# qwerfdsaplking/SATrans

Hardware: AMD Instinct MI355X
Metric: training samples/sec (AliCCP-shaped, emb=32, 3L/4H, meta_mode=QK) (higher is better)
Workload: dtype f32; 1 GPU; BASELINE configs[1]: AliCCP-shaped SATrans training step, 19 fields, 6,571,961 table rows (841 MB fp32), uniform ids, dropout on, dense-Adam+L2 semantics over all rows; batch_per_gpu=8192, global_batch=8192, embedding_dim=32, layers=3, heads=4, fields=19, parallelism=dp1

## Files before the change

include/satrans_hip.h:

```cpp
#ifndef SATRANS_HIP_H
#define SATRANS_HIP_H

#include <stdint.h>

#ifdef __cplusplus
extern "C" {
#endif

#define SATRANS_ABI_VERSION 7

#define SATRANS_OK 0
#define SATRANS_E_BADARG (-1)
#define SATRANS_E_UNSUPPORTED (-2)
#define SATRANS_E_LAUNCH (-3)
#define SATRANS_E_WORKSPACE (-4)

#define SATRANS_ID_F32 0
#define SATRANS_ID_I32 1
#define SATRANS_ID_I64 2

#define SATRANS_META_Q 1
#define SATRANS_META_K 2
#define SATRANS_RELU_OUT 4
#define SATRANS_NO_RES 8
// ... 129 lines not shown
    int64_t tab_stride;
    const float* x;
    const int32_t *order, *seg;
    const float *tab, *ln_g, *ln_b;
} satrans_metanet_desc;
int64_t satrans_metanet_saved_floats(const satrans_metanet_desc* d);
int64_t satrans_metanet_scratch_floats(const satrans_metanet_desc* d);
int satrans_metanet_fwd(const satrans_metanet_desc* d, float* y, float* saved, void* stream);
int satrans_metanet_bwd(const satrans_metanet_desc* d, const float* dy, float* dx, const float* saved, float* scratch,
                        float* g_tab, float* g_ln, void* stream);

int64_t satrans_layer_bwd_slab_floats(const satrans_layer_desc* d);
int satrans_layer_bwd(const satrans_layer_desc* d, const float* dy, float* dx, float* slabs,
                      float* g_wq, float* g_wk, float* g_wv, float* g_wo, float* g_ln, float* g_lnq,
                      float* g_lnk, float* g_tab_q, float* g_tab_k, void* stream);

int satrans_head(const float* a, const float* dense, int64_t dense_stride, const int32_t* dense_cols, int n_dense,
                 int B, int FD, const float* w, const float* bias, float* prob, float* logit, const float* y,
                 double* loss_sum, float* da, float* g_w, float* g_b, float* scratch, void* stream);

#define SATRANS_LOSS_BCE 0
#define SATRANS_LOSS_MSE 1
#define SATRANS_LOSS_MAE 2
int satrans_head_loss(const float* a, const float* dense, int64_t dense_stride, const int32_t* dense_cols, int n_dense, int B,
                      int FD, const float* w, const float* bias, float* prob, float* logit, const float* y, double* loss_sum,
                      float* da, float* g_w, float* g_b, float* scratch, int loss_kind, void* stream);

typedef struct satrans_head_desc {
    const float* w;
    const float* bias;
// ... 70 lines not shown
int satrans_embed_mark_touched(const int32_t* sorted_rows, int64_t n, int64_t total_rows, uint32_t* touched,
                               void* stream);

int satrans_embed_segment_sums(const int32_t* sorted_rows, const int32_t* src, int64_t n, const float* gemb, int D,
                               float* partial_ws, double* reg_partials, float* g_rows, void* stream);
int64_t satrans_embed_adam_rows_partials(int64_t rows, int D);
int satrans_embed_adam_rows(float* arena, float* m, float* v, int32_t* last, int64_t row0, int64_t rows, int D,
                            const float* g_rows, const satrans_adam_hparams* h, int t, double* reg_partials,
                            void* stream);
int satrans_embed_pack_rows(const int32_t* src, int64_t n, const float* gemb, int D, float* out, void* stream);

int64_t satrans_embed_lazy_reg_partials(int64_t n, int D);
int satrans_embed_lazy_replay(float* arena, float* m, float* v, int32_t* last, int D, const int32_t* sorted_rows,
                              int64_t n, int target, const double* table, const satrans_adam_hparams* h,
                              double* reg_partials, void* stream);
int satrans_embed_lazy_flush(float* arena, float* m, float* v, int32_t* last, int64_t total_rows, int D, int target,
                             const double* table, const satrans_adam_hparams* h, int64_t n, double* reg_partials,
                             void* stream);
int satrans_embed_lazy_mark(const int32_t* sorted_rows, int64_t n, int32_t* last, int t, void* stream);

int satrans_debug_check_packed_math(int mode, uint64_t first, uint64_t count, uint64_t* mismatches, void* stream);

int satrans_embed_grad_dense(const float* arena, const int32_t* sorted_rows, const int32_t* src, int64_t n,
                             const float* gemb, int64_t total_rows, int D, float l2, float* g_arena,
                             void* stream);

int satrans_sum_f64(const double* v, int64_t count, double* out, int accumulate, void* stream);

int64_t satrans_attn_stats_workspace_bytes(int B, int H, int F, int K);
int satrans_attn_stats_accumulate(const float* att, const int32_t* key, int B, int H, int F, int K, double* acc,
// ... 40 lines not shown
```

satrans_amd/csrc/capi.hip:

```cpp
#include <stdarg.h>
#include <stdlib.h>
#include <string.h>

#include "common.h"

namespace satrans {
static thread_local char g_error[512] = "";
void set_error(const char* fmt, ...) {
    va_list ap;
    va_start(ap, fmt);
    vsnprintf(g_error, sizeof(g_error), fmt, ap);
    va_end(ap);
}
static int g_layer_impl = -1;
}

extern "C" {

int satrans_layer_validate(const satrans_layer_desc* d, const char* who);
int satrans_layer_fused_supported(const satrans_layer_desc* d);
int satrans_layer_fwd_fused(const satrans_layer_desc* d, float* y, float* att, void* stream);
int satrans_layer_fwd_lds(const satrans_layer_desc* d, float* y, float* att, void* stream);
int satrans_layer_bwd_fused_supported(const satrans_layer_desc* d);
int64_t satrans_layer_bwd_slab_floats_fused(const satrans_layer_desc* d);
int64_t satrans_layer_attn_save_floats_fused(const satrans_layer_desc* d);
int satrans_layer_bwd_fused(const satrans_layer_desc* d, const float* dy, float* dx, float* slabs, float* g_wq, float* g_wk,
                            float* g_wv, float* g_wo, float* g_ln, float* g_lnq, float* g_lnk, float* g_tab_q,
                            float* g_tab_k, void* stream);
int64_t satrans_layer_bwd_slab_floats_lds(const satrans_layer_desc* d);
int satrans_layer_bwd_lds(const satrans_layer_desc* d, const float* dy, float* dx, float* slabs, float* g_wq, float* g_wk,
                          float* g_wv, float* g_wo, float* g_ln, float* g_lnq, float* g_lnk, float* g_tab_q,
                          float* g_tab_k, void* stream);

int satrans_layer_bwd_head_fused_supported(const satrans_layer_desc* d, const satrans_head_desc* h);
int64_t satrans_layer_bwd_head_scratch_floats_fused(const satrans_layer_desc* d, int n_dense);
int satrans_layer_bwd_head_fused(const satrans_layer_desc* d, const satrans_head_desc* h, float* dx, float* slabs, float* g_wq,
                                 float* g_wk, float* g_wv, float* g_wo, float* g_ln, float* g_lnq, float* g_lnk, float* g_tab_q,
                                 float* g_tab_k, void* stream);

// ... 48 lines not shown
                    "layer_fwd: SATRANS_X_SORTED / SATRANS_Y_SORTED are flags of the general path (satrans_layer_fwd_generic)");
    if (satrans_layer_impl() == 0 && satrans_layer_fused_supported(d)) return satrans_layer_fwd_fused(d, y, att, stream);
    return satrans_layer_fwd_lds(d, y, att, stream);
}

int64_t satrans_layer_bwd_slab_floats(const satrans_layer_desc* d) {
    if (satrans_layer_validate(d, "layer_bwd")) return -1;
    int64_t n = satrans_layer_bwd_slab_floats_lds(d);
    if (satrans_layer_bwd_fused_supported(d)) {
        const int64_t f = satrans_layer_bwd_slab_floats_fused(d);
        if (f > n) n = f;
    }
    return n;
}

int64_t satrans_layer_attn_save_floats(const satrans_layer_desc* d) {
    if (satrans_layer_validate(d, "layer_attn_save")) return -1;
    if (satrans_layer_impl() != 0 || !satrans_layer_fused_supported(d) || !satrans_layer_bwd_fused_supported(d)) return 0;
    return satrans_layer_attn_save_floats_fused(d);
}

int satrans_layer_bwd(const satrans_layer_desc* d, const float* dy, float* dx, float* slabs, float* g_wq, float* g_wk,
                      float* g_wv, float* g_wo, float* g_ln, float* g_lnq, float* g_lnk, float* g_tab_q, float* g_tab_k,
                      void* stream) {
    int rc = satrans_layer_validate(d, "layer_bwd");
    if (rc) return rc;
    SATRANS_REQUIRE(!(d->flags & (SATRANS_X_SORTED | SATRANS_Y_SORTED)), SATRANS_E_UNSUPPORTED,
                    "layer_bwd: SATRANS_X_SORTED / SATRANS_Y_SORTED are flags of the general path (satrans_layer_bwd_generic)");
    if (satrans_layer_impl() == 0 && satrans_layer_bwd_fused_supported(d))
        return satrans_layer_bwd_fused(d, dy, dx, slabs, g_wq, g_wk, g_wv, g_wo, g_ln, g_lnq, g_lnk, g_tab_q, g_tab_k, stream);
// ... 57 lines not shown
```

satrans_amd/csrc/embed_adam.hip:

```cpp
#include <algorithm>
#include <cstdlib>
#include <cstring>

#include <rocprim/rocprim.hpp>

#include "common.h"

namespace satrans {

constexpr int kChunk = 16;
constexpr int kStreamBlock = 256;
constexpr int kStreamBlocks = 2048;

struct AdamK {
    float neg_step, w1, beta2, w2, eps, l2x2, l2;
    double rbc2;
    float rbc2f;
    int fast;
};

__host__ inline AdamK make_adamk(const satrans_adam_hparams& h) {
    AdamK k;
    k.neg_step = -h.lr_over_bc1;
    k.rbc2 = 1.0 / (double)h.bc2_sqrt;
// ... 621 lines not shown
                reg = replay_element4(p, m, v, from, target, table, k);
                P[at] = p; M[at] = m; V[at] = v;
            }
        }
    }
    __syncthreads();
    if (j < n && c == 0) {
        const int32_t row = sorted_rows[j];
        if ((j == 0 || sorted_rows[j - 1] != row) && last[row] < target) last[row] = target;
    }
    const double total = block_sum(reg, s_red);
    if (threadIdx.x == 0) {
        reg_partials[blockIdx.x] = total;
        for (int64_t t = (int64_t)blockIdx.x + gridDim.x; t < slots; t += gridDim.x) reg_partials[t] = 0.0;
    }
}

template <int D>
__global__ __launch_bounds__(256) void lazy_flush_kernel(float4* __restrict__ P, float4* __restrict__ M, float4* __restrict__ V,
                                                        int32_t* __restrict__ last, int64_t total_rows, int target,
                                                        const double2* __restrict__ table, LazyK k,
                                                        double* __restrict__ reg_partials) {
    constexpr int LR = D / 4;
    __shared__ double s_red[256];
    double reg = 0.0;
    const int64_t groups_per_pass = (int64_t)gridDim.x * 256 / LR;
    const int c = threadIdx.x % LR;
    for (int64_t row = ((int64_t)blockIdx.x * 256 + threadIdx.x) / LR; row < total_rows; row += groups_per_pass) {
        const int from = last[row];
        if (from < target) {
// ... 630 lines not shown
    hipStream_t stream = (hipStream_t)stream_;
    SATRANS_REQUIRE(arena && m && v && last && sorted_rows && table && h && reg_partials, SATRANS_E_BADARG,
                    "embed_lazy_replay: null pointer");
    SATRANS_REQUIRE(n > 0 && target >= 0, SATRANS_E_BADARG, "embed_lazy_replay: n=%lld target=%d", (long long)n, target);
    const LazyK k = make_lazyk(*h);
    SATRANS_REQUIRE(D % 4 == 0, SATRANS_E_UNSUPPORTED, "embed_lazy_replay: embedding_dim %d is not a multiple of 4", D);
    const int64_t slots = ceil_div(n * D, 256);
    const int64_t blocks = ceil_div(n * (D / 4), 256);
    DISPATCH_D(D, (lazy_replay_kernel<DD><<<(unsigned)blocks, 256, 0, stream>>>((float4*)arena, (float4*)m, (float4*)v, last,
                                                                                sorted_rows, n, target, (const double2*)table, k,
                                                                                reg_partials, slots)));
    SATRANS_CHECK_LAUNCH("lazy_replay_kernel");
    return SATRANS_OK;
}

extern "C" int satrans_embed_lazy_flush(float* arena, float* m, float* v, int32_t* last, int64_t total_rows, int D,
                                        int target, const double* table, const satrans_adam_hparams* h, int64_t n,
                                        double* reg_partials, void* stream_) {
    hipStream_t stream = (hipStream_t)stream_;
    SATRANS_REQUIRE(arena && m && v && last && table && h && reg_partials, SATRANS_E_BADARG, "embed_lazy_flush: null pointer");
    const LazyK k = make_lazyk(*h);
    double* reg = reg_partials + ceil_div(n * D, 256);
    DISPATCH_D(D, (lazy_flush_kernel<DD><<<kFlushBlocks, 256, 0, stream>>>((float4*)arena, (float4*)m, (float4*)v, last, total_rows,
                                                                          target, (const double2*)table, k, reg)));
    SATRANS_CHECK_LAUNCH("lazy_flush_kernel");
    return SATRANS_OK;
}

extern "C" int satrans_debug_check_packed_math(int mode, uint64_t first, uint64_t count, uint64_t* mismatches, void* stream_) {
    hipStream_t stream = (hipStream_t)stream_;
// ... 53 lines not shown
```

satrans_amd/csrc/layer_fused.hip:

```cpp
#include <hip/hip_ext.h>

#include "layer_fused_common.h"

namespace satrans {

struct KernelTimer {
    static constexpr int kPairs = 512;
    struct Pair { hipEvent_t start, stop; int kind; };
    Pair pairs[kPairs];
    int made = 0, used = 0;
    bool armed = false;
    Pair* next(int kind) {
        if (!armed || used >= kPairs) return nullptr;
        if (used >= made) {
            if (hipEventCreate(&pairs[made].start) != hipSuccess || hipEventCreate(&pairs[made].stop) != hipSuccess) return nullptr;
            ++made;
        }
        pairs[used].kind = kind;
        return &pairs[used++];
    }
};
static KernelTimer g_ktimer;

#ifdef SATRANS_DIAG_FWDSAVE
// ... 1943 lines not shown
    const int LD = D + 4, LU = U + 4;
    auto r4 = [](int64_t v) { return (v + 3) & ~(int64_t)3; };
    const int64_t tasks = (int64_t)T * H * F;
    const int copies = tr ? 2 : 1;
    const int64_t dd = (int64_t)D * LD;
    const int64_t mlp = (int64_t)D * LU + (int64_t)U * LD;
    const int64_t hd = head ? r4((int64_t)F * D + kHeadDenseMax) + 64 + 64 + 128 + (int64_t)kFusedBlock * 4 * (D / 16) + 64 * kHeadDenseMax : 0;
    const int64_t FP = (F + 3) & ~3;
    const int64_t ds = std::max<int64_t>(std::max<int64_t>(tasks * F, 2 * (int64_t)T * F * D), (int64_t)T * H * FP * FP);
    return copies * 4 * dd + (same_tab ? 1 : 2) * copies * mlp + 6 * D + 5 * 64 * LD + 2 * r4(tasks) + r4(tasks * F) + r4(ds) + hd + 64;
}

static int fused_width(const satrans_layer_desc* d) { return d->D == 64 ? 16 : 2 * d->D; }

struct FusedBwdPlan {
    int T, G;
    size_t lds;
    bool tr;
};

static bool fused_bwd_plan(const satrans_layer_desc* d, FusedBwdPlan& p, bool head = false) {
    if (!satrans_layer_fused_supported(d) || d->D > 32 || d->F > 32) return false;
    const bool same_tab = d->tab_q == d->tab_k && d->lnq_g == d->lnk_g && d->lnq_b == d->lnk_b;
    p.T = 64 / d->F;
    p.tr = false;
    const int Uw = fused_width(d);
    p.lds = (size_t)fused_bwd_lds_floats(p.T, d->F, d->D, Uw, d->H, same_tab, p.tr, head) * 4;
    if (p.lds > 160 * 1024) return false;
    const int64_t tiles = ceil_div(d->B, p.T) + d->S;
    p.G = (int)std::max<int64_t>(1, std::min<int64_t>(tiles, cu_count()));
    return true;
}

template <int D, int U, int H, bool SAME, bool TR, int FT = 0, int MOD = 0, bool SAVE = false, bool HEADF = false>
static int launch_bwd(const satrans_layer_desc* d, const FusedBwdPlan& p, const float* dy, float* dx, float* slabs,
                      hipStream_t stream, const FusedHeadArgs* hd = nullptr) {
    static size_t attr_set = 0;
    if (p.lds > attr_set) {
        hipError_t e = hipFuncSetAttribute((const void*)layer_bwd_fused_kernel<D, U, H, SAME, TR, FT, MOD, SAVE, HEADF>,
                                           hipFuncAttributeMaxDynamicSharedMemorySize, (int)p.lds);
        SATRANS_REQUIRE(e == hipSuccess, SATRANS_E_LAUNCH, "layer_bwd(fused): LDS attribute: %s", hipGetErrorString(e));
        attr_set = p.lds;
    }
    if (KernelTimer::Pair* tp = g_ktimer.next(HEADF ? 2 : 1))
        hipExtLaunchKernelGGL((layer_bwd_fused_kernel<D, U, H, SAME, TR, FT, MOD, SAVE, HEADF>), dim3(p.G), dim3(kFusedBlock),
// ... 39 lines not shown

extern "C" int satrans_layer_bwd_fused_supported(const satrans_layer_desc* d) {
    FusedBwdPlan p;
    return d && fused_bwd_plan(d, p) ? 1 : 0;
}

extern "C" int64_t satrans_layer_attn_save_floats_fused(const satrans_layer_desc* d) {
    FusedBwdPlan p;
    if (!d || !fused_bwd_plan(d, p)) return 0;
    const bool alt = d->flags & (SATRANS_GATE | SATRANS_BILINEAR);
    if (d->D != 32 || (!alt && (d->U != 64 || !(d->flags & (SATRANS_META_Q | SATRANS_META_K))))) return 0;
    const int64_t HF = (int64_t)d->H * d->F;
    if (d->F > 32 || (d->F * HF) % 4 != 0) return 0;
    const int64_t FPs = (d->F + 3) & ~3;
    return (int64_t)d->B * ((int64_t)d->H * d->F * FPs + 2 * HF + (int64_t)d->F * d->D + (int64_t)d->F * (2 * d->D + 2));
}

extern "C" int64_t satrans_layer_bwd_slab_floats_fused(const satrans_layer_desc* d) {
    FusedBwdPlan p;
    if (!d) return -1;
    int64_t n = -1;
    if (fused_bwd_plan(d, p)) {
        const int64_t CSZ = 4 * (int64_t)d->D * d->D + 6 * d->D, TSZ = 4 * (int64_t)d->D * fused_width(d);
        n = std::max<int64_t>(n, (int64_t)p.G * CSZ + (int64_t)(p.G + d->S) * TSZ);
    }
    return n;
}

static int launch_fused_reduce(const satrans_layer_desc* d, const FusedBwdPlan& p, float* slabs, float* g_wq, float* g_wk,
                               float* g_wv, float* g_wo, float* g_ln, float* g_lnq, float* g_lnk, float* g_tab_q, float* g_tab_k,
// ... 229 lines not shown
```

satrans_amd/engine.py:

```python
from __future__ import annotations

import contextlib
import ctypes as C
import math
import os
from typing import Dict, List, Optional

import torch

from . import native as N
from .inputs import split_columns


from .engine_local import LocalStepMixin
from .engine_owner import OwnerStepMixin
from .engine_replicated import ReplicatedStepMixin
from .streams import _STREAMS, shared_stream as _shared_stream


class PathEngine(LocalStepMixin, ReplicatedStepMixin, OwnerStepMixin):
    def __init__(self, model):
        self.lib = N.lib()
        m = self.m = model
        self.dev = m.embedding_arena.device
# ... 142 lines not shown
        self._owner_world = 0
        self._replicas_stale = False
        self.reg_small = torch.zeros(1, dtype=torch.float64, device=self.dev)
        self.fuse_gather = not self.varlen
        self.fuse_head = True
        self.prefetch = True
        self.owner_prefetch = os.environ.get("SATRANS_OWNER_PREFETCH", "0") == "1"
        self.adam_arith = os.environ.get("SATRANS_ADAM_ARITH", "fast")
        if self.adam_arith not in ("fast", "exact"):
            raise ValueError(f"SATRANS_ADAM_ARITH={self.adam_arith!r}: 'fast' or 'exact'")
        self.untimed_phases = frozenset()
        self.prep_early = True
        self.defer_reduce = True
        self.side_tail = True
        self.preclear = True
        self._side_tail = None
        self._tail_done = None
        self._prep = None
        self.save_attention = True
        self.fwd_bf16 = os.environ.get("SATRANS_FWD_BF16", "0") == "1"
        self.force_split = os.environ.get("SATRANS_SPLIT_TABLES", "0") == "1"
        self.last_step = None
        self._hp_table = None
        self._hp_cfg = None
        self._lazy_pending = False

    def _stream(self):
        return N.stream_handle(self.dev)

    class _Phase:
# ... 677 lines not shown
                n = len(d_descs)
                descs_a = (C.POINTER(N.LayerDesc) * n)(*[C.pointer(d_) for d_ in d_descs])
                slabs_a = (C.c_void_p * n)(*d_slabs)
                grads_a = (N.LayerGrads * n)()
                for i_, gp in enumerate(d_grads):
                    for name_, v_ in zip(("g_wq", "g_wk", "g_wv", "g_wo", "g_ln", "g_lnq", "g_lnk", "g_tab_q", "g_tab_k"), gp):
                        setattr(grads_a[i_], name_, v_)
                with self.phase("layer_bwd_reduce"):
                    N.check(lib.satrans_layer_bwd_reduce(n, descs_a, slabs_a, grads_a, C.byref(d_head) if d_head is not None else None,
                                                         self._stream()), "satrans_layer_bwd_reduce")
            if modulated:
                with self.phase("scenario_bwd"):
                    self.scenario_tables_backward(g_tabs)

        fork = None
        if after_layers is not None or (side_tail and d_descs):
            fork = torch.cuda.Event()
            fork.record(torch.cuda.current_stream(self.dev))
        if after_layers is not None:
            after_layers(fork)
        self._last_fork = fork
        self._tail_done = None
        if side_tail and d_descs:
            main = torch.cuda.current_stream(self.dev)
            if self._side_tail is None:
                self._side_tail = _shared_stream(self.dev, "tail", lambda: torch.cuda.Stream(self.dev))
            self._side_tail.wait_event(fork)
            with torch.cuda.stream(self._side_tail):
                if clear_late and not precleared:
                    g_clear.zero_()
                finish()
                self._tail_done = torch.cuda.Event()
                self._tail_done.record(self._side_tail)
        else:
            if clear_late and not precleared:
# ... 14 lines not shown

    def _low_priority_stream(self, name: str = "low_priority"):
        def make():
            handle = C.c_void_p()
            with torch.cuda.device(self.dev):
                rc = self.lib.satrans_stream_create_low_priority(C.byref(handle))
            if rc == 0 and handle.value:
                return torch.cuda.ExternalStream(handle.value, device=self.dev)
            return None
        st = _shared_stream(self.dev, name, make)
        if st is not None or name != "low_priority":
            return st
        self.prep_early = False
        return _shared_stream(self.dev, "side", lambda: torch.cuda.Stream(self.dev))

    def _prepare_async(self, X_next, ws_cur_B, fork=None, defer_bucket=False):
        B = X_next.shape[0]
        ws = self.train_workspace(B, 1, False)
        if "prep_alt" not in ws:
            ws["prep_alt"] = {k: torch.empty_like(ws[k]) for k in self._PREP_KEYS}
        alt = ws["prep_alt"]
        main = torch.cuda.current_stream(self.dev)
        if self._side is None:
            self._side = self._low_priority_stream() if self.prep_early else \
                _shared_stream(self.dev, "side", lambda: torch.cuda.Stream(self.dev))
        if fork is None:
            fork = torch.cuda.Event()
            fork.record(main)
        self._side.wait_event(fork)
        with torch.cuda.stream(self._side):
            st = self._stream()
            f_, lo_, n_ = self._sort_fields
            N.check(self.lib.satrans_embed_rows_sort_fields(X_next.data_ptr(), N.id_dtype_of(X_next), X_next.stride(0),
                                                            self.cols.data_ptr(), self.row_span.data_ptr(), alt["rows"].data_ptr(),
                                                            B, self.F, f_, lo_, n_, alt["sorted_rows"].data_ptr(),
                                                            alt["src"].data_ptr(), self.status.data_ptr(), st),
                    "satrans_embed_rows_sort_fields(next)")
            sorted_ev = torch.cuda.Event()
            sorted_ev.record(self._side)
            done = None
            if not defer_bucket:
                self._bucket(X_next, alt)
                done = torch.cuda.Event()
                done.record(self._side)
        self._prep = dict(key=self._prep_key(X_next), X=X_next, B=B, done=done, sorted=sorted_ev)

    def _take_prepared(self, X, ws) -> bool:
        prep, self._prep = self._prep, None
        if prep is None:
            return False
        if prep["key"] != self._prep_key(X) or prep["B"] != X.shape[0] or "prep_alt" not in ws:
            torch.cuda.current_stream(self.dev).wait_event(prep["done"] or prep["sorted"])
            return False
        alt = ws["prep_alt"]
        for k in self._PREP_KEYS:
            ws[k], alt[k] = alt[k], ws[k]
        torch.cuda.current_stream(self.dev).wait_event(prep["sorted"])
        self._prep_rest = prep["done"] or prep["sorted"]
        return True

    def _join_prepared(self) -> None:
        ev, self._prep_rest = getattr(self, "_prep_rest", None), None
        if ev is not None:
            torch.cuda.current_stream(self.dev).wait_event(ev)

    def train_step(self, X: torch.Tensor, y: torch.Tensor, next_X: Optional[torch.Tensor] = None):
        from . import parallel
        X = self._prepare_input(X)
        y = y.reshape(-1).to(torch.float32).contiguous()
        B = X.shape[0]
        self._ensure_train_state()
# ... 16 lines not shown

    def _sort_rows(self, ws, B, rows, n, out_rows, out_src, touched, per_field=False):
        lib = self.lib
        if per_field and self._sort_fields is not None and touched is None and n == B * self.R and B <= 8192:
            f_, lo_, n_ = self._sort_fields
            N.check(lib.satrans_embed_sort_fields(rows.data_ptr(), B, self.F, f_, lo_, n_, out_rows.data_ptr(),
                                                  out_src.data_ptr(), self._stream()), "satrans_embed_sort_fields")
            return
        N.check(lib.satrans_embed_sort(rows.data_ptr(), n, self.total_rows, out_rows.data_ptr(), out_src.data_ptr(),
                                       touched, ws["sort_ws"].data_ptr(), ws["sort_ws"].numel(),
                                       ws["iota"].data_ptr(), self._stream()),
                "satrans_embed_sort")

    def _replay_rows(self, sorted_rows, n, reg, reg_sum):
        m, lib = self.m, self.lib
        table = self._table(self.adam_t)
        h = self._hparams(m.l2_reg_embedding)
        N.check(lib.satrans_embed_lazy_replay(m.embedding_arena.data_ptr(), self.adam_m.data_ptr(), self.adam_v.data_ptr(),
                                              self.last_step.data_ptr(), self.D, sorted_rows.data_ptr(), n,
                                              self.adam_t - 1, table.data_ptr(), C.byref(h), reg.data_ptr(),
                                              self._stream()), "satrans_embed_lazy_replay")
        if reg_sum is not None:
            N.check(lib.satrans_sum_f64(reg.data_ptr(), reg.numel(), reg_sum.data_ptr(), 1, self._stream()),
                    "satrans_sum_f64")

    def _rows_sorted(self, X, ws, B, st):
        lib, m = self.lib, self.m
        if self._sort_fields is not None and B <= 8192:
            f_, lo_, n_ = self._sort_fields
            with self.phase("embed_sort"):
# ... 134 lines not shown
            self._hp_table = torch.from_numpy(np.stack([col0, col1], axis=1)).to(self.dev).contiguous()
            self._hp_cfg = betas
            self._table_dirty = None
        elif dirty is not None:
            cap = self._hp_table.shape[0]
            col0 = np.float32(self._rates(dirty, cap) / self._hp_bc1[dirty:]).astype(np.float64)
            if dirty == 0:
                col0[0] = 0.0
            self._hp_table[dirty:, 0].copy_(torch.from_numpy(col0))
            self._table_dirty = None
        return self._hp_table

    def flush_lazy(self, sync: bool = True):
        self._join_flat()
        self._join_roll()
        if self.lazy and self._lazy_pending:
            m = self.m
            h = self._hparams(m.l2_reg_embedding) if self.adam_t > 0 else None
            st = self._stream()
            table = self._table(self.adam_t)
            with self.phase("lazy_flush"):
                self._flush_launches(m, h, st, table)
            self._lazy_pending = False
            self._since_flush = 0
            self.flush_count = getattr(self, "flush_count", 0) + 1
            self._prune_lr_history()
        if sync and self._replicas_stale:
            from . import parallel
            if sync == "local" and parallel.world_size() > 1:
                raise RuntimeError("the embedding tables of this rank are stale outside the slice it owns (data-parallel owner "
# ... 85 lines not shown
```

satrans_amd/engine_local.py:

```python
from __future__ import annotations

import contextlib
import ctypes as C

import torch

from . import native as N
from .streams import shared_stream


class LocalStepMixin:
    def _train_step_local(self, X, y, B, cfg, next_X=None):
        ws = self.train_workspace(B, 1, False)
        lib, m, D = self.lib, self.m, self.D
        main = torch.cuda.current_stream(self.dev)
        st = self._stream()
        split = self.force_split
        small_rows = self.small_rows if split else 0
        n_loc = B * self.R
        n_s = B * self.F_small if split else 0
        n_b = n_loc - n_s
        l2 = m.l2_reg_embedding
        arena, am, av = m.embedding_arena.data_ptr(), self.adam_m.data_ptr(), self.adam_v.data_ptr()

        prepared = self._take_prepared(X, ws)
        if not prepared:
            self._rows_sorted(X, ws, B, st)
        self.adam_t += 1
        self._note_lr(cfg["lr"])
        h_emb = self._hparams(l2)
        self._join_roll()
        if self.lazy and self.adam_t > 1:
            with self.phase("lazy_replay"):
                self._replay_rows(ws["sorted_rows"], n_loc, ws["replay_reg"], None)
        elif self.lazy:
            ws["replay_reg"].zero_()
        rolling = self.rolling_flush if self.lazy and self.flush_every > 1 and not split else ""
        rolled = False
        if rolling == "step":
            fork = torch.cuda.Event()
            fork.record(main)
            rolled = self._roll_flush(fork)
        side_done = None
        big_sorted, big_src = ws["sorted_rows"][n_s:], ws["src"][n_s:]
        if not self.lazy:
            use_side = self.overlap
            if use_side:
# ... 7 lines not shown
                                                       ws["touched"].data_ptr(), self._stream()),
                        "satrans_embed_mark_touched")
                if self.total_rows > small_rows:
                    with self.phase("adam_untouched"):
                        N.check(lib.satrans_embed_adam_untouched(arena, am, av, small_rows, self.total_rows, D,
                                                                 ws["touched"].data_ptr(), C.byref(h_emb),
                                                                 ws["reg_partials"].data_ptr(), 0, self._stream()),
                                "satrans_embed_adam_untouched")
                if use_side:
                    side_done = torch.cuda.Event()
                    side_done.record(self._side)

        hook = None
        if next_X is not None and self._dense_override is None and self._can_prepare(next_X, next_X.shape[0]) \
                and next_X.shape[1] >= self.n_cols:
            hook = lambda fork: self._prepare_async(next_X, B, fork)
        gemb = self.backward(X, y, ws, rows_ready=True, bucket_ready=prepared, after_layers=hook,
                             side_tail=self.side_tail and not split)
        if rolling and rolling != "step":
            rolled = self._roll_flush(self._last_fork)

        if n_s > 0:
            with self.phase("adam_small"):
                N.check(lib.satrans_embed_segment_sums(ws["sorted_rows"].data_ptr(), ws["src"].data_ptr(), n_s,
                                                       gemb.data_ptr(), D, ws["partial_ws"].data_ptr(),
                                                       ws["reg_unused"].data_ptr(), self.g_small.data_ptr(), st),
                        "satrans_embed_segment_sums")
        if small_rows > 0:
            self._small_tables_step(ws, small_rows, h_emb, st)
        if side_done is not None:
            main.wait_event(side_done)
# ... 37 lines not shown
```

satrans_amd/native.py:

```python
from __future__ import annotations

import ctypes as C
import os
import subprocess
from typing import Optional

import torch

os.environ.setdefault("GPU_MAX_HW_QUEUES", "8")

_HERE = os.path.dirname(os.path.abspath(__file__))
LIB_PATH = os.environ.get("SATRANS_LIB_PATH") or os.path.join(_HERE, "libsatrans_hip.so")
ABI_VERSION = 7

ID_F32, ID_I32, ID_I64 = 0, 1, 2
META_Q, META_K, RELU_OUT, NO_RES, TRAIN, GATE, BILINEAR = 1, 2, 4, 8, 16, 32, 64
X_SORTED, Y_SORTED = 128, 256

_c_f32p = C.c_void_p
_vp = C.c_void_p


class LayerDesc(C.Structure):
    _fields_ = [
# ... 98 lines not shown
    "satrans_layer_generic_saved_floats": (C.c_int64, [C.POINTER(LayerDesc)]),
    "satrans_layer_generic_scratch_floats": (C.c_int64, [C.POINTER(LayerDesc)]),
    "satrans_layer_fwd_generic": (C.c_int, [C.POINTER(LayerDesc), _vp, _vp, _vp, _vp]),
    "satrans_layer_bwd_generic": (C.c_int, [C.POINTER(LayerDesc), _vp, _vp, _vp, _vp, _vp, _vp, _vp, _vp, _vp, _vp, _vp, _vp,
                                            _vp, _vp]),
    "satrans_set_generic_attention": (C.c_int, [C.c_int]),
"satrans_selfatt_saved_floats": (C.c_int64, [C.POINTER(SelfAttDesc)]),
    "satrans_selfatt_scratch_floats": (C.c_int64, [C.POINTER(SelfAttDesc)]),
    "satrans_selfatt_fwd": (C.c_int, [C.POINTER(SelfAttDesc), _vp, _vp, _vp, _vp]),
    "satrans_selfatt_bwd": (C.c_int, [C.POINTER(SelfAttDesc), _vp, _vp, _vp, _vp, _vp, _vp, _vp, _vp, _vp, _vp]),
    "satrans_metanet_saved_floats": (C.c_int64, [C.POINTER(MetaNetDesc)]),
    "satrans_metanet_scratch_floats": (C.c_int64, [C.POINTER(MetaNetDesc)]),
    "satrans_metanet_fwd": (C.c_int, [C.POINTER(MetaNetDesc), _vp, _vp, _vp]),
    "satrans_metanet_bwd": (C.c_int, [C.POINTER(MetaNetDesc), _vp, _vp, _vp, _vp, _vp, _vp, _vp]),
    "satrans_layer_bwd_slab_floats": (C.c_int64, [C.POINTER(LayerDesc)]),
    "satrans_layer_attn_save_floats": (C.c_int64, [C.POINTER(LayerDesc)]),
    "satrans_batch_metrics": (C.c_int, [_vp, _vp, C.c_int, _vp, _vp]),
    "satrans_layer_bwd": (C.c_int, [C.POINTER(LayerDesc), _vp, _vp, _vp, _vp, _vp, _vp, _vp, _vp, _vp, _vp, _vp,
                                    _vp, _vp]),
    "satrans_layer_bwd_head_supported": (C.c_int, [C.POINTER(LayerDesc), C.POINTER(HeadDesc)]),
    "satrans_layer_bwd_head_scratch_floats": (C.c_int64, [C.POINTER(LayerDesc), C.c_int]),
    "satrans_layer_bwd_head": (C.c_int, [C.POINTER(LayerDesc), C.POINTER(HeadDesc), _vp, _vp, _vp, _vp, _vp, _vp, _vp, _vp, _vp,
                                         _vp, _vp, _vp]),
    "satrans_layer_bwd_deferred_supported": (C.c_int, [C.POINTER(LayerDesc)]),
    "satrans_layer_bwd_launch": (C.c_int, [C.POINTER(LayerDesc), _vp, _vp, _vp, _vp]),
    "satrans_layer_bwd_head_launch": (C.c_int, [C.POINTER(LayerDesc), C.POINTER(HeadDesc), _vp, _vp, _vp]),
    "satrans_layer_bwd_reduce": (C.c_int, [C.c_int, C.POINTER(C.POINTER(LayerDesc)), C.POINTER(_vp), C.POINTER(LayerGrads),
                                           C.POINTER(HeadDesc), _vp]),
    "satrans_head_scratch_floats": (C.c_int64, [C.c_int, C.c_int, C.c_int]),
    "satrans_head": (C.c_int, [_vp, _vp, C.c_int64, _vp, C.c_int, C.c_int, C.c_int, _vp, _vp, _vp, _vp, _vp, _vp,
# ... 22 lines not shown
    "satrans_embed_mark_touched": (C.c_int, [_vp, C.c_int64, C.c_int64, _vp, _vp]),
    "satrans_embed_segment_sums": (C.c_int, [_vp, _vp, C.c_int64, _vp, C.c_int, _vp, _vp, _vp, _vp]),
    "satrans_embed_adam_rows_partials": (C.c_int64, [C.c_int64, C.c_int]),
    "satrans_embed_adam_rows": (C.c_int, [_vp, _vp, _vp, _vp, C.c_int64, C.c_int64, C.c_int, _vp, C.POINTER(AdamHParams),
                                          C.c_int, _vp, _vp]),
    "satrans_embed_pack_rows": (C.c_int, [_vp, C.c_int64, _vp, C.c_int, _vp, _vp]),
    "satrans_embed_rows_sort_fields": (C.c_int, [_vp, C.c_int, C.c_int64, _vp, _vp, _vp, C.c_int, C.c_int, C.POINTER(C.c_int32),
                                                 C.POINTER(C.c_int32), C.POINTER(C.c_int32), _vp, _vp, _vp, _vp]),
    "satrans_embed_merge_runs": (C.c_int, [_vp, C.c_int64, C.POINTER(C.c_int64), C.c_int, _vp, _vp, _vp]),
    "satrans_embed_inverse_positions": (C.c_int, [_vp, C.c_int64, _vp, _vp]),
    "satrans_embed_sort_fields": (C.c_int, [_vp, C.c_int, C.c_int, C.POINTER(C.c_int32), C.POINTER(C.c_int32), C.POINTER(C.c_int32),
                                            _vp, _vp, _vp]),
    "satrans_embed_lazy_reg_partials": (C.c_int64, [C.c_int64, C.c_int]),
    "satrans_embed_lazy_replay": (C.c_int, [_vp, _vp, _vp, _vp, C.c_int, _vp, C.c_int64, C.c_int, _vp,
                                            C.POINTER(AdamHParams), _vp, _vp]),
    "satrans_embed_lazy_flush": (C.c_int, [_vp, _vp, _vp, _vp, C.c_int64, C.c_int, C.c_int, _vp, C.POINTER(AdamHParams),
                                           C.c_int64, _vp, _vp]),
    "satrans_embed_lazy_mark": (C.c_int, [_vp, C.c_int64, _vp, C.c_int, _vp]),
    "satrans_debug_check_packed_math": (C.c_int, [C.c_int, C.c_uint64, C.c_uint64, C.POINTER(C.c_uint64), _vp]),
    "satrans_embed_grad_dense": (C.c_int, [_vp, _vp, _vp, C.c_int64, _vp, C.c_int64, C.c_int, C.c_float, _vp, _vp]),
    "satrans_sum_f64": (C.c_int, [_vp, C.c_int64, _vp, C.c_int, _vp]),
    "satrans_attn_stats_workspace_bytes": (C.c_int64, [C.c_int, C.c_int, C.c_int, C.c_int]),
    "satrans_attn_stats_accumulate": (C.c_int, [_vp, _vp, C.c_int, C.c_int, C.c_int, C.c_int, _vp, _vp, C.c_int64, _vp]),
    "satrans_attn_inst_workspace_bytes": (C.c_int64, [C.c_int, C.c_int, C.c_int]),
    "satrans_attn_inst_check_rules": (C.c_int, [C.POINTER(AttnRule), C.c_int, C.c_int]),
    "satrans_attn_inst_match": (C.c_int, [_vp, C.c_int, C.c_int, C.c_int, C.POINTER(AttnRule), C.c_int, _vp, C.c_int64, _vp,
                                          C.c_int64, _vp, _vp, _vp, C.c_int64, _vp]),
    "satrans_attn_inst_gather": (C.c_int, [_vp, C.c_int, C.c_int, C.c_int, _vp, C.c_int64, C.c_int64, _vp, C.c_int64, _vp, _vp,
                                           _vp, _vp, C.c_int64, C.c_int, _vp, _vp]),
}
# ... 88 lines not shown
```

Measured before the change: 8.896 million samples/s.

## Add optional replay-ahead of lazy Adam rows on side stream with undo

```diff
diff --git a/include/satrans_hip.h b/include/satrans_hip.h
--- a/include/satrans_hip.h
+++ b/include/satrans_hip.h
@@ -167,6 +167,7 @@
 int satrans_layer_bwd(const satrans_layer_desc* d, const float* dy, float* dx, float* slabs,
                       float* g_wq, float* g_wk, float* g_wv, float* g_wo, float* g_ln, float* g_lnq,
                       float* g_lnk, float* g_tab_q, float* g_tab_k, void* stream);
+int satrans_layer_bwd_grid(const satrans_layer_desc* d, int head, int* G, int* rounds);
 
 int satrans_head(const float* a, const float* dense, int64_t dense_stride, const int32_t* dense_cols, int n_dense,
                  int B, int FD, const float* w, const float* bias, float* prob, float* logit, const float* y,
@@ -267,6 +268,12 @@
 int satrans_embed_lazy_replay(float* arena, float* m, float* v, int32_t* last, int D, const int32_t* sorted_rows,
                               int64_t n, int target, const double* table, const satrans_adam_hparams* h,
                               double* reg_partials, void* stream);
+int satrans_embed_lazy_replay_except(float* arena, float* m, float* v, int32_t* last, int D, const int32_t* sorted_rows,
+                                     int64_t n, const int32_t* held_rows, int64_t n_held, int target, const double* table,
+                                     const satrans_adam_hparams* h, double* reg_partials, float* undo, int32_t* undo_from,
+                                     void* stream);
+int satrans_embed_lazy_replay_undo(float* arena, float* m, float* v, int32_t* last, int D, const int32_t* sorted_rows,
+                                   int64_t n, const float* undo, const int32_t* undo_from, void* stream);
 int satrans_embed_lazy_flush(float* arena, float* m, float* v, int32_t* last, int64_t total_rows, int D, int target,
                              const double* table, const satrans_adam_hparams* h, int64_t n, double* reg_partials,
                              void* stream);
diff --git a/satrans_amd/csrc/capi.hip b/satrans_amd/csrc/capi.hip
--- a/satrans_amd/csrc/capi.hip
+++ b/satrans_amd/csrc/capi.hip
@@ -23,6 +23,7 @@
 int satrans_layer_fwd_lds(const satrans_layer_desc* d, float* y, float* att, void* stream);
 int satrans_layer_bwd_fused_supported(const satrans_layer_desc* d);
 int64_t satrans_layer_bwd_slab_floats_fused(const satrans_layer_desc* d);
+int satrans_layer_bwd_grid_fused(const satrans_layer_desc* d, int head, int* G, int* rounds);
 int64_t satrans_layer_attn_save_floats_fused(const satrans_layer_desc* d);
 int satrans_layer_bwd_fused(const satrans_layer_desc* d, const float* dy, float* dx, float* slabs, float* g_wq, float* g_wk,
                             float* g_wv, float* g_wo, float* g_ln, float* g_lnq, float* g_lnk, float* g_tab_q,
@@ -101,6 +102,14 @@
     return n;
 }
 
+int satrans_layer_bwd_grid(const satrans_layer_desc* d, int head, int* G, int* rounds) {
+    int rc = satrans_layer_validate(d, "layer_bwd_grid");
+    if (rc) return rc;
+    SATRANS_REQUIRE(satrans_layer_bwd_grid_fused(d, head, G, rounds) == SATRANS_OK, SATRANS_E_UNSUPPORTED,
+                    "layer_bwd_grid: the fused backward is not built for this shape");
+    return SATRANS_OK;
+}
+
 int64_t satrans_layer_attn_save_floats(const satrans_layer_desc* d) {
     if (satrans_layer_validate(d, "layer_attn_save")) return -1;
     if (satrans_layer_impl() != 0 || !satrans_layer_fused_supported(d) || !satrans_layer_bwd_fused_supported(d)) return 0;
diff --git a/satrans_amd/csrc/embed_adam.hip b/satrans_amd/csrc/embed_adam.hip
--- a/satrans_amd/csrc/embed_adam.hip
+++ b/satrans_amd/csrc/embed_adam.hip
@@ -659,6 +659,70 @@
         reg_partials[blockIdx.x] = total;
         for (int64_t t = (int64_t)blockIdx.x + gridDim.x; t < slots; t += gridDim.x) reg_partials[t] = 0.0;
     }
+}
+
+template <int D>
+__global__ __launch_bounds__(256) void lazy_replay_except_kernel(float4* __restrict__ P, float4* __restrict__ M, float4* __restrict__ V,
+                                                                int32_t* __restrict__ last, const int32_t* __restrict__ sorted_rows,
+                                                                int64_t n, const int32_t* __restrict__ held, int64_t n_held,
+                                                                int target, const double2* __restrict__ table, LazyK k,
+                                                                double* __restrict__ reg_partials, int64_t slots,
+                                                                float4* __restrict__ undo, int32_t* __restrict__ undo_from) {
+    constexpr int LR = D / 4;
+    __shared__ double s_red[256];
+    const int64_t j = ((int64_t)blockIdx.x * 256 + threadIdx.x) / LR;
+    const int c = threadIdx.x % LR;
+    double reg = 0.0;
+    int32_t row = 0;
+    int from = -1;
+    if (j < n) {
+        row = sorted_rows[j];
+        if (j == 0 || sorted_rows[j - 1] != row) {
+            int64_t lo = 0, hi = n_held;
+            while (lo < hi) {
+                const int64_t mid = (lo + hi) >> 1;
+                if (held[mid] < row) lo = mid + 1; else hi = mid;
+            }
+            if (lo == n_held || held[lo] != row) {
+                const int was = last[row];
+                if (was < target) from = was;
+            }
+        }
+        if (from >= 0) {
+            const int64_t at = (int64_t)row * LR + c, u = j * LR + c, plane = n * LR;
+            float4 p = P[at], m = M[at], v = V[at];
+            undo[u] = p; undo[plane + u] = m; undo[2 * plane + u] = v;
+            reg = replay_element4(p, m, v, from, target, table, k);
+            P[at] = p; M[at] = m; V[at] = v;
+        }
+    }
+    __syncthreads();
+    if (j < n && c == 0) {
+        undo_from[j] = from;
+        if (from >= 0) last[row] = target;
+    }
+    const double total = block_sum(reg, s_red);
+    if (threadIdx.x == 0) {
+        reg_partials[blockIdx.x] = total;
+        for (int64_t t = (int64_t)blockIdx.x + gridDim.x; t < slots; t += gridDim.x) reg_partials[t] = 0.0;
+    }
+}
+
+template <int D>
+__global__ __launch_bounds__(256) void lazy_replay_undo_kernel(float4* __restrict__ P, float4* __restrict__ M, float4* __restrict__ V,
+                                                              int32_t* __restrict__ last, const int32_t* __restrict__ sorted_rows,
+                                                              int64_t n, const float4* __restrict__ undo,
+                                                              const int32_t* __restrict__ undo_from) {
+    constexpr int LR = D / 4;
+    const int64_t j = ((int64_t)blockIdx.x * 256 + threadIdx.x) / LR;
+    const int c = threadIdx.x % LR;
+    if (j >= n) return;
+    const int from = undo_from[j];
+    if (from < 0) return;
+    const int32_t row = sorted_rows[j];
+    const int64_t at = (int64_t)row * LR + c, u = j * LR + c, plane = n * LR;
+    P[at] = undo[u]; M[at] = undo[plane + u]; V[at] = undo[2 * plane + u];
+    if (c == 0) last[row] = from;
 }
 
 template <int D>
@@ -1319,6 +1383,39 @@
     return SATRANS_OK;
 }
 
+extern "C" int satrans_embed_lazy_replay_except(float* arena, float* m, float* v, int32_t* last, int D,
+                                                const int32_t* sorted_rows, int64_t n, const int32_t* held_rows, int64_t n_held,
+                                                int target, const double* table, const satrans_adam_hparams* h,
+                                                double* reg_partials, float* undo, int32_t* undo_from, void* stream_) {
+    hipStream_t stream = (hipStream_t)stream_;
+    SATRANS_REQUIRE(arena && m && v && last && sorted_rows && held_rows && table && h && reg_partials && undo && undo_from,
+                    SATRANS_E_BADARG, "embed_lazy_replay_except: null pointer");
+    SATRANS_REQUIRE(n > 0 && n_held >= 0 && target >= 1, SATRANS_E_BADARG, "embed_lazy_replay_except: n=%lld n_held=%lld target=%d",
+                    (long long)n, (long long)n_held, target);
+    const LazyK k = make_lazyk(*h);
+    SATRANS_REQUIRE(D % 4 == 0, SATRANS_E_UNSUPPORTED, "embed_lazy_replay_except: embedding_dim %d is not a multiple of 4", D);
+    const int64_t slots = ceil_div(n * D, 256);
+    const int64_t blocks = ceil_div(n * (D / 4), 256);
+    DISPATCH_D(D, (lazy_replay_except_kernel<DD><<<(unsigned)blocks, 256, 0, stream>>>(
+                      (float4*)arena, (float4*)m, (float4*)v, last, sorted_rows, n, held_rows, n_held, target, (const double2*)table, k,
+                      reg_partials, slots, (float4*)undo, undo_from)));
+    SATRANS_CHECK_LAUNCH("lazy_replay_except_kernel");
+    return SATRANS_OK;
+}
+
+extern "C" int satrans_embed_lazy_replay_undo(float* arena, float* m, float* v, int32_t* last, int D, const int32_t* sorted_rows,
+                                              int64_t n, const float* undo, const int32_t* undo_from, void* stream_) {
+    hipStream_t stream = (hipStream_t)stream_;
+    SATRANS_REQUIRE(arena && m && v && last && sorted_rows && undo && undo_from && n > 0, SATRANS_E_BADARG,
+                    "embed_lazy_replay_undo: bad arguments");
+    SATRANS_REQUIRE(D % 4 == 0, SATRANS_E_UNSUPPORTED, "embed_lazy_replay_undo: embedding_dim %d is not a multiple of 4", D);
+    const int64_t blocks = ceil_div(n * (D / 4), 256);
+    DISPATCH_D(D, (lazy_replay_undo_kernel<DD><<<(unsigned)blocks, 256, 0, stream>>>(
+                      (float4*)arena, (float4*)m, (float4*)v, last, sorted_rows, n, (const float4*)undo, undo_from)));
+    SATRANS_CHECK_LAUNCH("lazy_replay_undo_kernel");
+    return SATRANS_OK;
+}
+
 extern "C" int satrans_embed_lazy_flush(float* arena, float* m, float* v, int32_t* last, int64_t total_rows, int D,
                                         int target, const double* table, const satrans_adam_hparams* h, int64_t n,
                                         double* reg_partials, void* stream_) {
diff --git a/satrans_amd/csrc/layer_fused.hip b/satrans_amd/csrc/layer_fused.hip
--- a/satrans_amd/csrc/layer_fused.hip
+++ b/satrans_amd/csrc/layer_fused.hip
@@ -1981,7 +1981,7 @@
 static int fused_width(const satrans_layer_desc* d) { return d->D == 64 ? 16 : 2 * d->D; }
 
 struct FusedBwdPlan {
-    int T, G;
+    int T, G, rounds;
     size_t lds;
     bool tr;
 };
@@ -1994,8 +1994,9 @@
     const int Uw = fused_width(d);
     p.lds = (size_t)fused_bwd_lds_floats(p.T, d->F, d->D, Uw, d->H, same_tab, p.tr, head) * 4;
     if (p.lds > 160 * 1024) return false;
-    const int64_t tiles = ceil_div(d->B, p.T) + d->S;
-    p.G = (int)std::max<int64_t>(1, std::min<int64_t>(tiles, cu_count()));
+    const int64_t tiles = std::max<int64_t>(1, ceil_div(d->B, p.T) + d->S);
+    p.rounds = (int)ceil_div(tiles, cu_count());
+    p.G = (int)ceil_div(tiles, p.rounds);
     return true;
 }
 
@@ -2065,6 +2066,14 @@
     if (d->F > 32 || (d->F * HF) % 4 != 0) return 0;
     const int64_t FPs = (d->F + 3) & ~3;
     return (int64_t)d->B * ((int64_t)d->H * d->F * FPs + 2 * HF + (int64_t)d->F * d->D + (int64_t)d->F * (2 * d->D + 2));
+}
+
+extern "C" int satrans_layer_bwd_grid_fused(const satrans_layer_desc* d, int head, int* G, int* rounds) {
+    FusedBwdPlan p;
+    if (!d || !fused_bwd_plan(d, p, head != 0)) return SATRANS_E_UNSUPPORTED;
+    if (G) *G = p.G;
+    if (rounds) *rounds = p.rounds;
+    return SATRANS_OK;
 }
 
 extern "C" int64_t satrans_layer_bwd_slab_floats_fused(const satrans_layer_desc* d) {
diff --git a/satrans_amd/engine.py b/satrans_amd/engine.py
--- a/satrans_amd/engine.py
+++ b/satrans_amd/engine.py
@@ -180,6 +180,10 @@
         self.defer_reduce = True
         self.side_tail = True
         self.preclear = True
+        self.replay_ahead = os.environ.get("SATRANS_REPLAY_AHEAD", "0") == "1"
+        self._ahead = None
+        self._ahead_target = None
+        self.ahead_taken = self.ahead_undone = 0
         self._side_tail = None
         self._tail_done = None
         self._prep = None
@@ -887,11 +891,14 @@
                     self.scenario_tables_backward(g_tabs)
 
         fork = None
-        if after_layers is not None or (side_tail and d_descs):
+        if after_layers is not None or (side_tail and d_descs) or self._ahead is not None:
             fork = torch.cuda.Event()
             fork.record(torch.cuda.current_stream(self.dev))
         if after_layers is not None:
             after_layers(fork)
+        ahead, self._ahead = self._ahead, None
+        if ahead is not None:
+            ahead(fork)
         self._last_fork = fork
         self._tail_done = None
         if side_tail and d_descs:
@@ -936,7 +943,7 @@
         self.prep_early = False
         return _shared_stream(self.dev, "side", lambda: torch.cuda.Stream(self.dev))
 
-    def _prepare_async(self, X_next, ws_cur_B, fork=None, defer_bucket=False):
+    def _prepare_async(self, X_next, ws_cur_B, fork=None, defer_bucket=False, held=None):
         B = X_next.shape[0]
         ws = self.train_workspace(B, 1, False)
         if "prep_alt" not in ws:
@@ -966,17 +973,64 @@
                 done = torch.cuda.Event()
                 done.record(self._side)
         self._prep = dict(key=self._prep_key(X_next), X=X_next, B=B, done=done, sorted=sorted_ev)
+        if held is not None:
+            self._ahead = lambda ev: self._replay_ahead(ev, ws, alt, held)
+
+    def _replay_ahead(self, fork, ws, alt, held):
+        prep, m, D = self._prep, self.m, self.D
+        n = alt["sorted_rows"].numel()
+        if "reg_partials" not in alt:
+            alt["reg_partials"] = torch.zeros_like(ws["reg_partials"])
+            alt["replay_reg"] = alt["reg_partials"][ws["reg_partials"].numel() - ws["replay_reg"].numel():]
+            ws["ahead_undo"] = torch.empty(3 * n * D, dtype=torch.float32, device=self.dev)
+            ws["ahead_from"] = torch.empty(n, dtype=torch.int32, device=self.dev)
+        h = self._hparams(m.l2_reg_embedding)
+        table = self._table(self.adam_t)
+        if fork is not None:
+            self._side.wait_event(fork)
+        with torch.cuda.stream(self._side):
+            N.check(self.lib.satrans_embed_lazy_replay_except(
+                m.embedding_arena.data_ptr(), self.adam_m.data_ptr(), self.adam_v.data_ptr(), self.last_step.data_ptr(), D,
+                alt["sorted_rows"].data_ptr(), n, held.data_ptr(), held.numel(), self.adam_t, table.data_ptr(), C.byref(h),
+                alt["replay_reg"].data_ptr(), ws["ahead_undo"].data_ptr(), ws["ahead_from"].data_ptr(), self._stream()),
+                "satrans_embed_lazy_replay_except")
+            done = torch.cuda.Event()
+            done.record(self._side)
+        prep["ahead"] = dict(done=done, target=self.adam_t, rows=alt["sorted_rows"], n=n, undo=ws["ahead_undo"],
+                             undo_from=ws["ahead_from"])
+
+    def _cancel_ahead(self, prep=None) -> None:
+        prep = self._prep if prep is None else prep
+        ahead = prep.pop("ahead", None) if prep else None
+        if ahead is None:
+            return
+        self.ahead_undone += 1
+        torch.cuda.current_stream(self.dev).wait_event(ahead["done"])
+        N.check(self.lib.satrans_embed_lazy_replay_undo(
+            self.m.embedding_arena.data_ptr(), self.adam_m.data_ptr(), self.adam_v.data_ptr(), self.last_step.data_ptr(), self.D,
+            ahead["rows"].data_ptr(), ahead["n"], ahead["undo"].data_ptr(), ahead["undo_from"].data_ptr(), self._stream()),
+            "satrans_embed_lazy_replay_undo")
 
     def _take_prepared(self, X, ws) -> bool:
         prep, self._prep = self._prep, None
+        self._ahead_target = None
         if prep is None:
             return False
         if prep["key"] != self._prep_key(X) or prep["B"] != X.shape[0] or "prep_alt" not in ws:
             torch.cuda.current_stream(self.dev).wait_event(prep["done"] or prep["sorted"])
+            self._cancel_ahead(prep)
             return False
         alt = ws["prep_alt"]
         for k in self._PREP_KEYS:
             ws[k], alt[k] = alt[k], ws[k]
+        ahead = prep.get("ahead")
+        if ahead is not None:
+            for k in ("reg_partials", "replay_reg"):
+                ws[k], alt[k] = alt[k], ws[k]
+            self._ahead_target = ahead["target"]
+            self.ahead_taken += 1
+            torch.cuda.current_stream(self.dev).wait_event(ahead["done"])
+            return True
         torch.cuda.current_stream(self.dev).wait_event(prep["sorted"])
         self._prep_rest = prep["done"] or prep["sorted"]
         return True
@@ -1023,6 +1077,7 @@
 
     def _replay_rows(self, sorted_rows, n, reg, reg_sum):
         m, lib = self.m, self.lib
+        self._cancel_ahead()
         table = self._table(self.adam_t)
         h = self._hparams(m.l2_reg_embedding)
         N.check(lib.satrans_embed_lazy_replay(m.embedding_arena.data_ptr(), self.adam_m.data_ptr(), self.adam_v.data_ptr(),
@@ -1187,6 +1242,7 @@
     def flush_lazy(self, sync: bool = True):
         self._join_flat()
         self._join_roll()
+        self._cancel_ahead()
         if self.lazy and self._lazy_pending:
             m = self.m
             h = self._hparams(m.l2_reg_embedding) if self.adam_t > 0 else None
diff --git a/satrans_amd/engine_local.py b/satrans_amd/engine_local.py
--- a/satrans_amd/engine_local.py
+++ b/satrans_amd/engine_local.py
@@ -30,7 +30,9 @@
         self._note_lr(cfg["lr"])
         h_emb = self._hparams(l2)
         self._join_roll()
-        if self.lazy and self.adam_t > 1:
+        if self.lazy and self._ahead_target is not None and self._ahead_target == self.adam_t - 1:
+            pass
+        elif self.lazy and self.adam_t > 1:
             with self.phase("lazy_replay"):
                 self._replay_rows(ws["sorted_rows"], n_loc, ws["replay_reg"], None)
         elif self.lazy:
@@ -68,7 +70,12 @@
         hook = None
         if next_X is not None and self._dense_override is None and self._can_prepare(next_X, next_X.shape[0]) \
                 and next_X.shape[1] >= self.n_cols:
-            hook = lambda fork: self._prepare_async(next_X, B, fork)
+            rolling_on = self.lazy and self.flush_every > 1 and not split and bool(self.rolling_flush)
+            held = None
+            if self.replay_ahead and self.lazy and not split and not rolling_on and \
+                    not (self.flush_every and self._since_flush + 1 >= self.flush_every):
+                held = ws["sorted_rows"]
+            hook = lambda fork: self._prepare_async(next_X, B, fork, held=held)
         gemb = self.backward(X, y, ws, rows_ready=True, bucket_ready=prepared, after_layers=hook,
                              side_tail=self.side_tail and not split)
         if rolling and rolling != "step":
diff --git a/satrans_amd/native.py b/satrans_amd/native.py
--- a/satrans_amd/native.py
+++ b/satrans_amd/native.py
@@ -136,6 +136,7 @@
     "satrans_metanet_fwd": (C.c_int, [C.POINTER(MetaNetDesc), _vp, _vp, _vp]),
     "satrans_metanet_bwd": (C.c_int, [C.POINTER(MetaNetDesc), _vp, _vp, _vp, _vp, _vp, _vp, _vp]),
     "satrans_layer_bwd_slab_floats": (C.c_int64, [C.POINTER(LayerDesc)]),
+    "satrans_layer_bwd_grid": (C.c_int, [C.POINTER(LayerDesc), C.c_int, C.POINTER(C.c_int), C.POINTER(C.c_int)]),
     "satrans_layer_attn_save_floats": (C.c_int64, [C.POINTER(LayerDesc)]),
     "satrans_batch_metrics": (C.c_int, [_vp, _vp, C.c_int, _vp, _vp]),
     "satrans_layer_bwd": (C.c_int, [C.POINTER(LayerDesc), _vp, _vp, _vp, _vp, _vp, _vp, _vp, _vp, _vp, _vp, _vp,
@@ -188,6 +189,9 @@
     "satrans_embed_lazy_reg_partials": (C.c_int64, [C.c_int64, C.c_int]),
     "satrans_embed_lazy_replay": (C.c_int, [_vp, _vp, _vp, _vp, C.c_int, _vp, C.c_int64, C.c_int, _vp,
                                             C.POINTER(AdamHParams), _vp, _vp]),
+    "satrans_embed_lazy_replay_except": (C.c_int, [_vp, _vp, _vp, _vp, C.c_int, _vp, C.c_int64, _vp, C.c_int64, C.c_int, _vp,
+                                                   C.POINTER(AdamHParams), _vp, _vp, _vp, _vp]),
+    "satrans_embed_lazy_replay_undo": (C.c_int, [_vp, _vp, _vp, _vp, C.c_int, _vp, C.c_int64, _vp, _vp, _vp]),
     "satrans_embed_lazy_flush": (C.c_int, [_vp, _vp, _vp, _vp, C.c_int64, C.c_int, C.c_int, _vp, C.POINTER(AdamHParams),
                                            C.c_int64, _vp, _vp]),
     "satrans_embed_lazy_mark": (C.c_int, [_vp, C.c_int64, _vp, C.c_int, _vp]),
```

After: 8.888 million samples/s. Within noise of the previous version (-0.1%).
